# strukturag/libde265

Hardware: AMD Instinct MI355X
Metric: decoded CTBs/s (higher is better)
Workload: dtype u16; 1 GPU; c5_8k10_8tiles; width=7680, height=4320, bit_depth=10, tiles=4x2, ctbs_per_picture=8160, stages=inter+residual+intra+deblock+sao, parallelism=pictures/1

## Files before the change

### libde265_amd/csrc/k_common.h

```cpp
#ifndef M355_K_COMMON_H
#define M355_K_COMMON_H

#include <hip/hip_runtime.h>
#include <stdint.h>

#include "de265_mi355x.h"
#include <k_asm.h>

struct DevRef {
  const void* plane[3];
  int stride[3];
  int valid;
  int pad;
};

struct DevIntraWork {
  uint32_t ctb;
  uint32_t ib_start, ib_count;
  uint16_t nb_same;
  uint16_t nb_earlier;
  uint8_t waves_code;
  uint8_t pad[3];
  uint32_t plan_base;
  uint32_t plan_count;
// ... 273 lines not shown
  uint32_t max_units, n;
  int32_t cf, nhwc, bf16, u16, bdl, bdc;
  float scale[3], bias[3];
  m355_rgb_coeffs k;
  ExportTensorRoi fr[M355_TENSOR_MAX_FRAMES];
  int32_t chroma_loc, pad;
  ColourArgs colour;
};
static_assert(sizeof(ExportTensorRoi) == 88 && sizeof(ExportTensorRoisArgs) <= 4096, "the records of a batch of regions must fit the kernel arguments");
void m355_launch_export_tensor_rois(const ExportTensorRoisArgs& a, int src_bytes, int elem_bytes, int filter, hipStream_t st);

template <class T> __device__ __forceinline__ T d_sel3(int c, T a0, T a1, T a2)
{
  M355_PIN_V(a0); M355_PIN_V(a1); M355_PIN_V(a2);
  return c == 0 ? a0 : (c == 1 ? a1 : a2);
}
#define M355_SEL3(arr, c) d_sel3((c), (arr)[0], (arr)[1], (arr)[2])

#define M355_GATE(p) do { if ((p).timeout[1] == (p).epoch) return; } while (0)

enum { E_TU_V = 1, E_TU_H = 2, E_PB_V = 4, E_PB_H = 8, E_NONZERO = 16 };

struct DevBatch { const DevPic* pics; uint32_t on; };
#define M355_BATCH_PIC_AT(b, k) if (!(((b).on >> (k)) & 1u)) return; const DevPic& p = (b).pics[(k)]
#define M355_BATCH_PIC(b) M355_BATCH_PIC_AT(b, blockIdx.z)
struct HostBatch { const DevPic* host; const DevPic* dev; int n; uint32_t on; };

void m355_launch_validate(const DevPic& p, hipStream_t st);
void m355_launch_meta(const DevPic& p, hipStream_t st);
void m355_launch_clear_gated(const DevPic& p, void* ptr, size_t bytes, hipStream_t st);
void m355_launch_meta_jobs(const DevPic& p, hipStream_t st);
void m355_launch_job_count(const DevPic& p, bool clear_planes, hipStream_t st);
void m355_launch_job_list(const DevPic& p, hipStream_t st);
void m355_launch_meta_planes(const DevPic& p, hipStream_t st, bool cleared, bool with_tu = true);
void m355_launch_meta_planes_jobs(const DevPic& p, hipStream_t st);
void m355_launch_tu_plan(const DevPic& p, hipStream_t st);
void m355_launch_inter(const DevPic& p, bool hbd, hipStream_t st);
#define M355_INTER_TAB_WORDS 300
void m355_inter_tables(bool bytes, int bd_luma, int bd_chroma, uint32_t* out);
void m355_launch_residual(const DevPic& p, bool hbd, bool big, hipStream_t st);
void m355_launch_residual_both(const DevPic& p, bool hbd, hipStream_t st);
void m355_launch_residual_add(const DevPic& p, bool hbd, hipStream_t st);
void m355_launch_residual_tu_plan(const DevPic& p, bool hbd, hipStream_t st);
void m355_launch_intra_plan(const DevPic& p, hipStream_t st);
void m355_launch_intra(const DevPic& p, bool hbd, hipStream_t st, bool ticket_zero = false);
void m355_launch_meta_planes_batch(const HostBatch& b, hipStream_t st);
void m355_launch_residual_batch(const HostBatch& b, bool hbd, bool big, hipStream_t st);
void m355_launch_intra_plan_batch(const HostBatch& b, hipStream_t st);
void m355_launch_deblock_batch(const HostBatch& b, bool hbd, hipStream_t st);
void m355_launch_sao_batch(const HostBatch& b, bool hbd, hipStream_t st);
void m355_launch_intra_batch(const DevPic& first, bool hbd, bool res32, const DevPic* dev_pics, int n, int max_work, uint32_t* ticket, int grid, hipStream_t st);
void m355_launch_deblock(const DevPic& p, bool hbd, hipStream_t st);
void m355_launch_deblock_pass(const DevPic& p, bool hbd, bool vertical, hipStream_t st);
void m355_launch_sao(const DevPic& p, bool hbd, hipStream_t st);
void m355_launch_halo_pack(const DevPic& p, const HaloLayout& h, bool hbd, int which, void* samples, uint32_t* meta, hipStream_t st);
void m355_launch_halo_add(uint32_t* buf, const uint32_t* scratch, uint32_t pitch_words, int n, uint32_t words, hipStream_t st);
void m355_launch_halo_unpack(const DevPic& p, const HaloLayout& h, bool hbd, int which, const void* samples, const uint32_t* meta, hipStream_t st);

__device__ __forceinline__ int d_clip3(int lo, int hi, int v) { return min(max(v, lo), hi); }
__device__ __forceinline__ int d_clip_bd(int v, int bd) { return d_clip3(0, (1 << bd) - 1, v); }
__device__ __forceinline__ int d_abs(int v) { return v < 0 ? -v : v; }
__device__ __forceinline__ int d_sign(int v) { return (v > 0) - (v < 0); }

__device__ __forceinline__ void wave_sync()
{
  __builtin_amdgcn_fence(__ATOMIC_RELEASE, "wavefront");
// ... 19 lines not shown
```

### libde265_amd/csrc/k_meta.hip

```cpp
#include <algorithm>
#include "k_common.h"
#include "k_meta_tu.h"
#include "record_checks.h"

__device__ __forceinline__ void k_meta_cu_body(const DevPic& p, const int blk)
{
  M355_GATE(p);
  const int i = blk * blockDim.x + threadIdx.x;
  if (i >= p.n_cus) return;
  const m355_cu cu = p.cus[i];
  const int x0 = cu.x, y0 = cu.y;
  const int l2m = p.pp.log2_min_cb_size;
  const int n = 1 << (cu.log2_size - l2m);
  const int cx = x0 >> l2m, cy = y0 >> l2m;
  for (int y = cy; y < cy + n && y < p.hcb; y++)
    for (int x = cx; x < cx + n && x < p.wcb; x++) p.cb_cu[y * p.wcb + x] = (uint32_t)i + 1;

  const int ctb_mask = (1 << p.pp.log2_ctb_size) - 1;
  const m355_slice sh = d_slice_at(p, x0, y0);
  int left = x0 != 0, top = y0 != 0;
  if (x0 && (x0 & ctb_mask) == 0) {
    if (!(sh.flags & M355_SF_LF_ACROSS_SLICES) && sh.slice_addr_rs != d_slice_at(p, x0 - 1, y0).slice_addr_rs) left = 0;
    else if (!(p.pp.flags & M355_PF_LF_ACROSS_TILES) && p.tile_id[d_ctb_of(p, x0, y0)] != p.tile_id[d_ctb_of(p, x0 - 1, y0)]) left = 0;
  }
// ... 46 lines not shown
}
__host__ __device__ static inline size_t d_meta_fill16(const DevPic& p) { return ((((size_t)2 * p.w4 * p.h4 + 63) & ~(size_t)63) + (size_t)p.wcb * p.hcb * 4 + 15) / 16; }
__global__ void __launch_bounds__(256) k_job_count(DevPic p, int clear_planes)
{
  M355_GATE(p);
  if (clear_planes) {
    if (blockIdx.x == 0 && threadIdx.x == 0) *p.ticket = 0;
    const size_t n16 = d_meta_fill16(p);
    uint4* q = (uint4*)p.edge_tu;
    for (size_t k = (size_t)blockIdx.x * 256 + threadIdx.x; k < n16; k += (size_t)gridDim.x * 256) q[k] = make_uint4(0, 0, 0, 0);
  }
  const int i = blockIdx.x * 256 + threadIdx.x;
  constexpr int NR = M355_JOB_RANGES;
  int cnt[NR] = {0, 0};
  if (i < p.n_pbs) {
    const m355_pb pb = p.pbs[i];
    const int rng = d_pb_range(p, pb);
    const int n = d_pb_jobs(pb);
#pragma unroll
    for (int k = 0; k < NR; k++) cnt[k] = rng == k ? n : 0;
  }
  __shared__ int s_w[4][NR];
#pragma unroll
  for (int k = 0; k < NR; k++) {
#pragma unroll
    for (int d = 32; d >= 1; d >>= 1) cnt[k] += __shfl_xor(cnt[k], d, 64);
  }
  if ((threadIdx.x & 63) == 0) {
#pragma unroll
    for (int k = 0; k < NR; k++) s_w[threadIdx.x >> 6][k] = cnt[k];
  }
  __syncthreads();
  if (threadIdx.x < NR) p.job_base[blockIdx.x * NR + threadIdx.x] = (uint32_t)(s_w[0][threadIdx.x] + s_w[1][threadIdx.x] + s_w[2][threadIdx.x] + s_w[3][threadIdx.x]);
}
__device__ __forceinline__ void k_meta_pb_body(const DevPic& p, const int chunk, const int n_chunks)
{
  constexpr int NR = M355_JOB_RANGES;
  const int i = chunk * 256 + (int)threadIdx.x;
  const int lane = threadIdx.x & 63;
  const bool active = i < p.n_pbs;
  m355_pb pb;
  if (active) pb = p.pbs[i]; else { pb.x = pb.y = 0; pb.w = pb.h = 0; pb.flags = 0; }
  const int ns = pb.w >> 2;
  const int njobs = active ? d_pb_jobs(pb) : 0;
  const int rng = !active ? NR : d_pb_range(p, pb);
  int incl[NR];
#pragma unroll
  for (int k = 0; k < NR; k++) incl[k] = rng == k ? njobs : 0;
#pragma unroll
  for (int d = 1; d < 64; d <<= 1) {
#pragma unroll
    for (int k = 0; k < NR; k++) { const int t = __shfl_up(incl[k], (unsigned)d, 64); if (lane >= d) incl[k] += t; }
  }
  __shared__ int s_wtot[4][NR];
  const int wave = threadIdx.x >> 6;
  if (lane == 63) {
#pragma unroll
    for (int k = 0; k < NR; k++) s_wtot[wave][k] = incl[k];
  }
  __syncthreads();
  __shared__ uint32_t s_red[4][2 * NR];
  {
    uint32_t acc[2 * NR] = {0, 0, 0, 0};
    for (int ch = (int)threadIdx.x; ch < n_chunks; ch += 256) {
#pragma unroll
      for (int k = 0; k < NR; k++) {
// ... 80 lines not shown
  const int l2w = p.pp.log2_ctb_size - csw, l2h = p.pp.log2_ctb_size - csh;
  const int xC = xCtb << l2w, yC = yCtb << l2h;
  const int ctbSliceAddrRS = d_slice_at(p, min(xC, p.pp.width - 1), min(yC, p.pp.height - 1)).slice_addr_rs;
  const int curFlags = p.slices[p.ctbs[ctb].slice_idx].flags;
  const bool across_tiles = (p.pp.flags & M355_PF_LF_ACROSS_TILES) != 0;
  uint32_t mask = 0;
  for (int k = 0; k < 9; k++) {
    const int nx = xCtb + k % 3 - 1, ny = yCtb + k / 3 - 1;
    bool blocked = true;
    if (nx >= 0 && ny >= 0 && nx < p.ctbW && ny < p.ctbH) {
      const int n = ny * p.ctbW + nx;
      const m355_slice shN = p.slices[p.ctbs[n].slice_idx];
      blocked = (shN.slice_addr_rs < ctbSliceAddrRS && !(curFlags & M355_SF_LF_ACROSS_SLICES)) ||
                (shN.slice_addr_rs > ctbSliceAddrRS && !(shN.flags & M355_SF_LF_ACROSS_SLICES)) ||
                (!across_tiles && p.tile_id[n] != p.tile_id[ctb]);
    }
    if (blocked) mask |= 1u << k;
  }
  if (curFlags & (c == 0 ? M355_SF_SAO_LUMA : M355_SF_SAO_CHROMA)) mask |= 0x8000u;
  p.sao_nb[i] = (uint16_t)mask;
}

void m355_launch_job_count(const DevPic& p, bool clear_planes, hipStream_t st)
{
  if (!p.n_pbs) return;
  hipLaunchKernelGGL(k_job_count, dim3((p.n_pbs + 255) / 256), dim3(256), 0, st, p, clear_planes ? 1 : 0);
}
void m355_launch_job_list(const DevPic& p, hipStream_t st)
{
  if (!p.n_pbs) return;
  const int n_chunks = (p.n_pbs + 255) / 256;
  hipLaunchKernelGGL(k_meta_pb, dim3(n_chunks), dim3(256), 0, st, p);
}
void m355_launch_meta_jobs(const DevPic& p, hipStream_t st)
{
  m355_launch_job_count(p, false, st);
  m355_launch_job_list(p, st);
}

__global__ void __launch_bounds__(256) k_meta_planes(DevPic p, int nb_cu)
{
  const int b = (int)blockIdx.x;
  if (b < nb_cu) k_meta_cu_body(p, b);
  else k_meta_sao_body(p, b - nb_cu);
}
__global__ void __launch_bounds__(256) k_meta_planes_jobs(DevPic p, int nb_pb, int nb_cu)
{
  M355_GATE(p);
  const int b = (int)blockIdx.x;
  if (b < nb_pb) k_meta_pb_body(p, b, nb_pb);
  else if (b < nb_pb + nb_cu) k_meta_cu_body(p, b - nb_pb);
  else k_meta_sao_body(p, b - nb_pb - nb_cu);
}
__global__ void __launch_bounds__(256) k_meta_tu(DevPic p) { k_meta_tu_body(p, (int)blockIdx.x); }
__global__ void __launch_bounds__(256) k_meta_cu_batch(DevBatch b) { M355_BATCH_PIC(b); k_meta_cu_body(p, (int)blockIdx.x); }
__global__ void __launch_bounds__(256) k_meta_tu_batch(DevBatch b) { M355_BATCH_PIC(b); k_meta_tu_body(p, (int)blockIdx.x); }
__global__ void __launch_bounds__(256) k_meta_sao_batch(DevBatch b) { M355_BATCH_PIC(b); k_meta_sao_body(p, (int)blockIdx.x); }
__global__ void __launch_bounds__(256) k_meta_fill_batch(DevBatch b)
{
  M355_BATCH_PIC(b);
  const size_t n16 = d_meta_fill16(p);
  uint4* q = (uint4*)p.edge_tu;
  for (size_t i = (size_t)blockIdx.x * 256 + threadIdx.x; i < n16; i += (size_t)gridDim.x * 256) q[i] = make_uint4(0, 0, 0, 0);
}

void m355_launch_meta_planes(const DevPic& p, hipStream_t st, bool cleared, bool with_tu)
// ... 82 lines not shown
```

### libde265_amd/csrc/runtime.hip

```cpp
#include "runtime_internal.h"

thread_local std::string g_err;
int fail(int code, const char* fmt, ...)
{
  char buf[512];
  va_list ap; va_start(ap, fmt); vsnprintf(buf, sizeof(buf), fmt, ap); va_end(ap);
  g_err = buf;
  return code;
}

extern "C" {
int ev_mark(m355_ctx* c, hipStream_t st, EvRef* out) {
  const unsigned long long t = ++c->ev_ticket;
  m355_ctx::EvSlot& e = c->evring[t % M355_EV_RING];
  if (!e.ev) { if (hipEventCreateWithFlags(&e.ev, hipEventDisableTiming) != hipSuccess) return fail(M355_ERR_HIP, "hipEventCreate failed"); }
  else if (e.ticket) hipEventSynchronize(e.ev);
  if (hipEventRecord(e.ev, st) != hipSuccess) return fail(M355_ERR_HIP, "hipEventRecord failed");
  e.ticket = t;
  out->ticket = t; out->stream = st;
  return M355_OK;
}
void ev_wait(m355_ctx* c, hipStream_t st, const EvRef& r) {
  if (!r.ticket || r.stream == st) return;
  const m355_ctx::EvSlot& e = c->evring[r.ticket % M355_EV_RING];
// ... 12 lines not shown

hipStream_t reader_begin(m355_ctx* c, Frame* f, int kind, const uint32_t** gate, uint32_t* epoch) {
  const hipStream_t st = f->wr_stream ? f->wr_stream : lane(c).stream;
  if (!f->wr_stream) ev_wait(c, st, f->wr);
  ev_wait(c, st, f->reader[kind]);
  if (!gate) return st;
  if (f->wr_stream && f->wr_gate) { *gate = f->wr_gate; *epoch = f->wr_epoch; }
  else {
    *gate = lane(c).timeout; *epoch = ++c->epoch;
    if (*epoch == 0) *epoch = ++c->epoch;
  }
  return st;
}
int reader_end(m355_ctx* c, Frame* f, int kind, hipStream_t st) { return ev_mark(c, st, &f->reader[kind]); }
void readers_wait(m355_ctx* c, hipStream_t st, const Frame* f) {
  for (const EvRef& m : f->reader) ev_wait(c, st, m);
}

int lane_class_priority(int index) {
  static int lo = 0, hi = 0, probed = 0;
  if (!probed) { probed = 1; if (hipDeviceGetStreamPriorityRange(&lo, &hi) != hipSuccess) lo = hi = 0; }
  const int cls = (index / 3) % 3;
  return cls == 0 ? 0 : (cls == 1 ? hi : lo);
}
int lane_priorities_mode() { return 2; }
static int lane_priority(int index) { return lane_priorities_mode() == 1 ? lane_class_priority(index) : 0; }
static int lane_create(m355_ctx* c, Lane& l, int index)
{
  HIPCHK(hipStreamCreateWithPriority(&l.stream, hipStreamNonBlocking, lane_priority(index)));
  HIPCHK(hipStreamCreateWithPriority(&l.stream2, hipStreamNonBlocking, lane_priority(index)));
  HIPCHK(hipEventCreateWithFlags(&l.ev_fork, hipEventDisableTiming));
  HIPCHK(hipEventCreateWithFlags(&l.ev_fork2, hipEventDisableTiming));
  HIPCHK(hipEventCreateWithFlags(&l.ev_join, hipEventDisableTiming));
  HIPCHK(hipMalloc(&l.ticket, 64));
  HIPCHK(hipMalloc(&l.timeout, 128));
  HIPCHK(hipMemsetAsync(l.ticket, 0, 64, l.stream));
  HIPCHK(hipMemsetAsync(l.timeout, 0, 128, l.stream));
  HIPCHK(hipMemsetAsync(l.timeout + 2, 0xFF, 8, l.stream));
  HIPCHK(hipStreamSynchronize(l.stream));
  return M355_OK;
}
static void lane_destroy(Lane& l)
{
  if (l.stream) hipStreamSynchronize(l.stream);
  if (l.stream2) hipStreamSynchronize(l.stream2);
  if (l.work.used) frame_free(l.work);
  void* bufs[] = {l.pb_of, l.edge, l.ticket, l.timeout, l.edge_tu, l.cuf, l.resbuf, l.jobs, l.sao_nb, l.iplan, l.job_base};
  for (void* b : bufs) if (b) hipFree(b);
  if (l.ev_fork) hipEventDestroy(l.ev_fork);
  if (l.ev_fork2) hipEventDestroy(l.ev_fork2);
  if (l.ev_join) hipEventDestroy(l.ev_join);
  if (l.stream_hi) { hipStreamSynchronize(l.stream_hi); hipStreamDestroy(l.stream_hi); }
  if (l.stream2) hipStreamDestroy(l.stream2);
  if (l.stream) hipStreamDestroy(l.stream);
  l = Lane();
}
hipError_t sync_all(m355_ctx* c) {
  hipError_t e = hipSuccess;
  auto sync = [&](hipStream_t s) { if (s) { hipError_t e2 = hipStreamSynchronize(s); if (e == hipSuccess) e = e2; } };
  for (const Lane& l : c->lanes) { sync(l.stream); sync(l.stream_hi); }
  for (hipStream_t bs : c->batch_stream) sync(bs);
  sync(c->maps_stream);
  return e;
}


static std::vector<TileRect> rank_tiles(const m355_pic_params& pp, int rank, int nranks)
{
  std::vector<TileRect> v;
  const int cs = 1 << pp.log2_ctb_size, n_tiles = pp.num_tile_cols * pp.num_tile_rows;
  for (int ty = 0, t = 0; ty < pp.num_tile_rows; ty++)
    for (int tx = 0; tx < pp.num_tile_cols; tx++, t++) {
      if (m355_shard_owner_of_tile(t, n_tiles, nranks) != rank) continue;
      TileRect r = {pp.col_bd[tx] * cs, pp.row_bd[ty] * cs, pp.col_bd[tx + 1] * cs, pp.row_bd[ty + 1] * cs};
      if (r.x1 > pp.width) r.x1 = pp.width;
      if (r.y1 > pp.height) r.y1 = pp.height;
      v.push_back(r);
    }
  return v;
}
static size_t tiles_bytes(const m355_pic_params& pp, const std::vector<TileRect>& v)
{
  const int cf = pp.chroma_format_idc;
  const int sw = (cf == 1 || cf == 2) ? 2 : 1, sh = cf == 1 ? 2 : 1;
// ... 933 lines not shown
```

### libde265_amd/csrc/runtime_decode.hip

```cpp
#include "runtime_internal.h"

extern "C" {

bool chain_residuals_forced();

int prepare(m355_ctx* c, Resident& r, DevPic& d_out, bool& want_sao_out, hipStream_t st) {
  hipSetDevice(c->device);
  const m355_picture& pic = r.hdr;
  const m355_pic_params& pp = pic.pp;
  Frame* dst = get_frame(c, pic.dst_frame);
  if (!dst) return fail(M355_ERR_INVALID, "dst_frame %d is not a live frame", pic.dst_frame);
  if (dst->w != pp.width || dst->h != pp.height || dst->cf != pp.chroma_format_idc || dst->bdl != pp.bit_depth_luma || dst->bdc != pp.bit_depth_chroma)
    return fail(M355_ERR_INVALID, "dst frame geometry does not match the picture parameters");
  DevPic d = r.dp;
  d.ref_valid = 0;
  DevRef refs[M355_MAX_REF_FRAMES];
  memset(refs, 0, sizeof(refs));
  for (int i = 0; i < M355_MAX_REF_FRAMES; i++) {
    if (pic.ref_frames[i] < 0) continue;
    Frame* f = get_frame(c, pic.ref_frames[i]);
    if (!f) return fail(M355_ERR_INVALID, "ref_frames[%d]=%d is not a live frame", i, pic.ref_frames[i]);
    if (f->w != dst->w || f->h != dst->h || f->cf != dst->cf || f->bdl != dst->bdl || f->bdc != dst->bdc)
      return fail(M355_ERR_INVALID, "reference frame %d geometry differs (motion.cc:377-398 would conceal; record FILL instead)", i);
    if (f == dst) return fail(M355_ERR_INVALID, "a picture cannot reference itself");
    for (int cc = 0; cc < 3; cc++) { refs[i].plane[cc] = f->plane[cc]; refs[i].stride[cc] = f->stride[cc]; }
    refs[i].valid = 1;
    d.ref_valid |= 1u << i;
  }
  if (!r.refs_dev) {
    HIPCHK(hipMalloc(&r.refs_dev, sizeof(refs)));
    HIPCHK(hipHostMalloc(&r.refs_host, sizeof(refs), hipHostMallocDefault));
    r.refs_valid = false;
  }
  if (!r.refs_valid || memcmp(r.refs_host, refs, sizeof(refs)) != 0) {
    if (!r.fresh) HIPCHK(sync_all(c));
    memcpy(r.refs_host, refs, sizeof(refs));
    HIPCHK(hipMemcpyAsync(r.refs_dev, r.refs_host, sizeof(refs), hipMemcpyHostToDevice, st));
// ... 5 lines not shown
    const uint32_t* tab = nullptr;
    for (auto& e : c->inter_tabs) if (e.first == key) tab = e.second;
    if (!tab) {
      uint32_t host[M355_INTER_TAB_WORDS];
      m355_inter_tables(dst->bpp[0] == 1, std::min((int)pp.bit_depth_luma, 16), std::min((int)pp.bit_depth_chroma, 16), host);
      uint32_t* dev = nullptr;
      HIPCHK(hipMalloc(&dev, sizeof(host)));
      HIPCHK(hipMemcpy(dev, host, sizeof(host), hipMemcpyHostToDevice));
      c->inter_tabs.emplace_back(key, dev);
      tab = dev;
    }
    d.inter_tabs = tab;
  }
  Lane& L = lane(c);
  int rc;
  {
    const size_t u4 = (size_t)d.w4 * d.h4, ncb = (size_t)d.wcb * d.hcb;
    const size_t need = ((2 * u4 + 63) & ~(size_t)63) + ncb * 4 + 64;
    if ((rc = grow(&L.edge_tu, &L.cap_u4, need, st, false))) return rc;
    if ((rc = grow(&L.pb_of, &L.cap_cb, u4, st, true))) return rc;
  }
  {
    size_t n = 0;
    for (int cc = 0; cc < 3; cc++) {
      d.edge_col_ofs[cc] = (uint32_t)n; n += (size_t)d.ctbW * (size_t)(dst->ph[cc] >> 1);
      d.edge_row_ofs[cc] = (uint32_t)n; n += (size_t)d.ctbH * (size_t)(dst->pw[cc] >> 1);
    }
    if ((rc = grow(&L.edge, &L.cap_edge, n + 1, st, true))) return rc;
  }
  if ((rc = grow(&L.cuf, &L.cap_cuf, (size_t)pic.n_cus + (size_t)r.halo.n_units + 1, st, false))) return rc;
  const size_t res_intra = (((size_t)pic.res_len + 64) & ~(size_t)63) * (m355_res32(pp) ? 2 : 1);
  size_t res_tiles = 0;
  for (int s = 0; s < 4; s++) { d.res_tile_base[s] = (uint32_t)res_tiles; res_tiles += (size_t)pic.rb_count[s] << (2 * (s + 2)); }
  const bool tiles = (c->depth >= sched::chain_residual_tiles_min_depth || chain_residuals_forced()) && (long long)pic.pp.width * pic.pp.height <= sched::one_stream_max_samples;
  const size_t res_need = res_intra + (tiles ? res_tiles : 0) + 1;
  if ((rc = grow(&L.resbuf, &L.cap_res, res_need, st, false))) return rc;
  d.res_tiles = tiles ? L.resbuf + res_intra : nullptr;
  d.res_front = 0;
  if ((rc = grow(&L.sao_nb, &L.cap_sao, (size_t)d.nCtb * 3, st, false))) return rc;
  {
    const size_t area = (size_t)pp.width * pp.height;
    const size_t cap = pic.n_pbs > 0 ? std::min(area / 16, area / 32 + 8 * (size_t)pic.n_pbs) + 256 : 1;
    const size_t n_chunks = ((size_t)(pic.n_pbs > 0 ? pic.n_pbs : 0) + 255) / 256;
    if ((rc = grow(&L.jobs, &L.cap_jobs, cap, st, false))) return rc;
    if ((rc = grow(&L.job_base, &L.cap_jobbase, n_chunks * M355_JOB_RANGES + 8, st, true))) return rc;
    d.jobs_cap = (uint32_t)cap; d.job_base = L.job_base; d.job_tot = L.job_base + n_chunks * M355_JOB_RANGES;
  }
  if ((rc = grow(&L.iplan, &L.cap_iplan, (size_t)r.n_iplan + 8, st, false))) return rc;

  const bool want_sao = (c->stages & M355_STAGE_SAO) && (pp.flags & M355_PF_SAO_ENABLED);
  Frame* target = dst;
  if (want_sao) {
    if (!L.work.used || L.work.w != dst->w || L.work.h != dst->h || L.work.cf != dst->cf || L.work.bdl != dst->bdl || L.work.bdc != dst->bdc) {
      HIPCHK(sync_all(c));
      if (L.work.used) frame_free(L.work);
      frame_geometry(L.work, dst->w, dst->h, dst->cf, dst->bdl, dst->bdc);
      if ((rc = frame_alloc(L.work, st))) return rc;
    }
    target = &L.work;
  }
  for (int cc = 0; cc < 3; cc++) {
    d.pw[cc] = dst->pw[cc]; d.ph[cc] = dst->ph[cc];
    d.plane[cc] = target->plane[cc]; d.stride[cc] = target->stride[cc];
    d.out_plane[cc] = dst->plane[cc]; d.out_stride[cc] = dst->stride[cc];
  }
  d.edge_tu = L.edge_tu; d.edge_pb = L.edge_tu + (size_t)d.w4 * d.h4;
  d.cb_cu = (uint32_t*)(L.edge_tu + (((size_t)2 * d.w4 * d.h4 + 63) & ~(size_t)63));
  d.cuf = L.cuf; d.pb_of = L.pb_of;
  d.fill_pb_of_in_meta = ((c->stages & M355_STAGE_INTER) && m355_inter_uses_jobs(d)) ? 0 : 1;
  d.jobs = L.jobs; d.sao_nb = L.sao_nb; d.iplan = L.iplan;
  d.resbuf = L.resbuf; d.edge = L.edge; d.ticket = L.ticket; d.timeout = L.timeout;
  {
    static const int grid_env = getenv("M355_INTRA_GRID") ? atoi(getenv("M355_INTRA_GRID")) : 0;
    static int slots = 0;
    if (!slots) { hipDeviceProp_t prop; slots = (hipGetDeviceProperties(&prop, c->device) == hipSuccess && prop.multiProcessorCount > 0) ? 2 * prop.multiProcessorCount : 512; }
    d.intra_grid = grid_env > 0 ? grid_env : std::max(64, slots / std::max(1, c->depth));
    d.intra_keeper = c->depth <= sched::intra_keeper_max_depth;
    if (!d.intra_keeper && r.dp.intra_dense) {
      bool idle = true;
      for (int i = 0; i < c->depth && idle; i++) if (&c->lanes[i] != &L && ev_query(c, c->lanes[i].last) != hipSuccess) idle = false;
      d.intra_keeper = idle;
    }
    static const bool no_keeper = getenv("M355_TEST_NO_KEEPER") != nullptr;
    if (no_keeper) d.intra_keeper = 0;
    static const int halo_late = getenv("M355_TEST_HALO_LATE") ? atoi(getenv("M355_TEST_HALO_LATE")) : 0;
    d.test_halo_late = halo_late;
  }
  d.epoch = ++c->epoch;
  if (d.epoch == 0) d.epoch = ++c->epoch;
  c->dbg_intra[0] = r.n_intra_work; c->dbg_intra[1] = r.n_intra_ticket; c->dbg_intra[2] = r.n_intra_heavy; c->dbg_intra[3] = r.n_intra_light;
  d_out = d; want_sao_out = want_sao;
  return M355_OK;
}

void clear_target(m355_ctx* c, const DevPic& d, Frame* tgt, bool gated, hipStream_t st) {
  for (int cc = 0; cc < 3; cc++) {
    if (!tgt->pw[cc]) continue;
    const size_t bytes = (size_t)tgt->stride[cc] * tgt->ph[cc] * tgt->bpp[cc];
    if (gated) m355_launch_clear_gated(d, tgt->plane[cc], bytes, st);
    else hipMemsetAsync(tgt->plane[cc], 0, bytes, st);
  }
}

bool chain_residuals_forced() { static const bool on = getenv("M355_TEST_CHAIN_RESIDUALS") != nullptr; return on; }

hipStream_t launch_prediction(m355_ctx* c, const Resident& r, const DevPic& d, bool hbd, hipStream_t st, hipEvent_t* ev, bool with_intra, hipStream_t chain, Frame* hazard_dst) {
  Lane& L = lane(c);
  const bool single = d.intra_dense || (long long)d.pp.width * d.pp.height <= sched::one_stream_max_samples;
  hipStream_t s2 = single ? st : L.stream2;
  static const int clear_min = getenv("M355_CLEAR_IN_COUNT_MIN") ? atoi(getenv("M355_CLEAR_IN_COUNT_MIN")) : sched::clear_in_count_min_pbs;
  const bool clear_in_count = d.n_pbs >= std::max(1, clear_min);
  bool tu_plan_with_residuals = false;
  const bool res_front = (chain || chain_residuals_forced()) && d.res_tiles && (c->stages & M355_STAGE_RESIDUAL) && d.pp.bit_depth_luma <= 15 && d.pp.bit_depth_chroma <= 15 &&
                         d.rb_count[0] + d.rb_count[1] + d.rb_count[2] + d.rb_count[3] > 0;
  if (clear_in_count) m355_launch_job_count(d, true, st);
  if (!single) { hipEventRecord(L.ev_fork, st); hipStreamWaitEvent(s2, L.ev_fork, 0); }
  if (single && clear_in_count && (c->stages & M355_STAGE_INTRA)) {
    m355_launch_meta_planes_jobs(d, st);
    if (c->depth <= sched::tu_plan_in_residuals_max_depth && (c->stages & M355_STAGE_RESIDUAL) && !res_front) tu_plan_with_residuals = true; else m355_launch_tu_plan(d, st);
  } else {
    if (c->stages & M355_STAGE_INTRA) {
      m355_launch_meta_planes(d, s2, clear_in_count, false);
      m355_launch_tu_plan(d, s2);
    } else m355_launch_meta_planes(d, s2, clear_in_count);
    if (clear_in_count) m355_launch_job_list(d, st); else m355_launch_meta_jobs(d, st);
  }
  auto launch_residuals = [&](const DevPic& dd) {
    hipStream_t sr = !single ? s2 : st;
    if (sr != st) { hipEventRecord(L.ev_fork2, st); hipStreamWaitEvent(s2, L.ev_fork2, 0); }
    if (tu_plan_with_residuals) m355_launch_residual_tu_plan(dd, hbd, st);
    else if (sr == st) m355_launch_residual_both(dd, hbd, st);
    else {
      m355_launch_residual(dd, hbd, false, sr);
      m355_launch_residual(dd, hbd, true, st);
    }
  };
  if (res_front) { DevPic dq = d; dq.res_front = 1; launch_residuals(dq); }
  if (ev) hipEventRecord(ev[1], st);
  if (chain && chain != st) {
    EvRef front;
    if (ev_mark(c, st, &front) == M355_OK) {
      st = chain; ev_wait(c, st, front);
      if (ev) hipEventRecord(ev[1], st);
    }
  }
  if (hazard_dst) dst_hazards(c, hazard_dst, true, st);
  if (c->depth >= 2)
    for (int i = 0; i < M355_MAX_REF_FRAMES; i++) {
      Frame* f = r.hdr.ref_frames[i] >= 0 ? get_frame(c, r.hdr.ref_frames[i]) : nullptr;
      if (f) ev_wait(c, st, f->wr);
    }
  if (c->stages & M355_STAGE_INTER) m355_launch_inter(d, hbd, st);
  if (ev) hipEventRecord(ev[2], st);
  if ((c->stages & M355_STAGE_RESIDUAL) && !res_front) launch_residuals(d);
  else if (res_front) m355_launch_residual_add(d, hbd, st);
  if (!single) { hipEventRecord(L.ev_join, s2); hipStreamWaitEvent(st, L.ev_join, 0); }
  if (ev) hipEventRecord(ev[3], st);
  if (with_intra && (c->stages & M355_STAGE_INTRA)) m355_launch_intra(d, hbd, st, clear_in_count);
  if (ev) hipEventRecord(ev[4], st);
  return st;
}

void dst_hazards(m355_ctx* c, Frame* dstf, bool piped, hipStream_t st) {
  readers_wait(c, st, dstf);
  if (!piped) return;
  ev_wait(c, st, dstf->wr);
  for (int k = 0; k < M355_MAX_LANES; k++) ev_wait(c, st, dstf->rd[k]);
}

int mark_done(m355_ctx* c, Resident& r, Frame* dstf, hipStream_t st, const DevPic* d) {
  const int rc = ev_mark(c, st, &r.done);
  if (rc) return rc;
  r.fresh = false;
  dstf->wr_stream = st; dstf->wr = r.done;
  dstf->wr_gate = d ? d->timeout : nullptr; dstf->wr_epoch = d ? d->epoch : 0;
  lane(c).last = r.done; lane(c).last_stream = st;
  return M355_OK;
}

struct DecodeState {
  DevPic d; bool want_sao = false; hipEvent_t* ev = nullptr;
  hipStream_t st = nullptr;
};

enum { PRE_ALL = 0, PRE_NO_INTRA = 1, PRE_HAZARDS = 2 };
static int decode_pre(m355_ctx* c, Resident& r, bool rotate, DecodeState& S, int mode, hipStream_t on_stream = nullptr)
{
  const bool with_intra = mode == PRE_ALL;
  if (r.sharded) return fail(M355_ERR_INVALID, "a sharded picture is decoded by phases (m355_decode_phase)");
  hipStream_t chain = nullptr;
  if (rotate && c->depth >= 2) {
// ... 94 lines not shown
  if (e != hipSuccess) return fail(M355_ERR_HIP, "kernel launch failed: %s", hipGetErrorString(e));
  {
    static const bool dbg = getenv("M355_DEBUG_TIMEOUT") && atoi(getenv("M355_DEBUG_TIMEOUT"));
    if (dbg) {
      hipStreamSynchronize(st);
      uint32_t t = 0;
      hipMemcpy(&t, lane(c).timeout, 4, hipMemcpyDeviceToHost);
      if (t) fprintf(stderr, "m355: decode %llu (epoch %u, %d pbs, %d ibs, %d cus, lane %d): intra wait gave up\n", c->serial, d.epoch, d.n_pbs, d.n_ibs, d.n_cus, c->active);
    }
  }
  return M355_OK;
}

int decode(m355_ctx* c, Resident& r, bool rotate) {
  DecodeState S;
  const int rc = decode_pre(c, r, rotate, S, PRE_ALL);
  return rc ? rc : decode_post(c, r, S);
}

int status_of(m355_ctx* c, m355_ctx::Status& s) {
  if (!s.validated) return M355_OK;
  const uint32_t* w = c->status_words + 4 * (s.serial % M355_STATUS_RING);
  if (w[1] != s.epoch) return M355_OK;
  const unsigned long long key = (unsigned long long)w[2] | ((unsigned long long)w[3] << 32);
  uint32_t bad = (uint32_t)key;
  if ((uint32_t)(key >> 32) != ~s.epoch) bad = 0;
  static const char* const names[8] = {"?", "cu", "tu", "pb", "weight", "rb", "ib", "?"};
  s.reported = true;
  return fail(M355_ERR_INVALID, "picture %llu: %s %u rejected by the device-side list validation (the picture was not decoded)", s.serial, names[(bad >> 28) & 7], bad & 0x0FFFFFFFu);
}

unsigned long long m355_last_serial(m355_ctx* c) { return c->serial; }
M355_API void m355_debug_intra_counts(m355_ctx* c, int* out) { for (int i = 0; i < 4; i++) out[i] = c->dbg_intra[i]; }

int m355_decode_status(m355_ctx* c, unsigned long long serial)
{
  if (serial == 0 || serial > c->serial) return fail(M355_ERR_INVALID, "no decode with serial %llu", serial);
  m355_ctx::Status& s = c->status[serial % M355_STATUS_RING];
  if (s.serial != serial) return fail(M355_ERR_STALE, "decode %llu is older than the last %d decodes: its status is no longer kept (m355_wait reports rejections)", serial, M355_STATUS_RING);
  hipSetDevice(c->device);
  const hipError_t q = ev_query(c, s.done);
  if (q == hipErrorNotReady) return M355_ERR_BUSY;
  if (q != hipSuccess) return fail(M355_ERR_HIP, "hipEventQuery failed: %s", hipGetErrorString(q));
  return status_of(c, s);
}

int m355_decode_batch(m355_ctx* c, const int* handles, int n)
{
  if (n < 1 || !handles) return fail(M355_ERR_INVALID, "m355_decode_batch: no pictures");
  if (n > std::max(1, c->depth)) return fail(M355_ERR_INVALID, "m355_decode_batch: %d pictures on %d lanes (m355_set_pipeline_depth)", n, c->depth);
  for (int k = 0; k < n; k++) {
    const int h = handles[k];
    if (h < 0 || h >= (int)c->resident.size() || !c->resident[h].used) return fail(M355_ERR_INVALID, "bad picture handle");
    for (int j = 0; j < k; j++) if (handles[j] == h) return fail(M355_ERR_INVALID, "m355_decode_batch: picture %d twice in one batch", h);
    const Resident& r = c->resident[h];
    const m355_pic_params &a = r.hdr.pp, &b = c->resident[handles[0]].hdr.pp;
    if (r.sharded) return fail(M355_ERR_INVALID, "a sharded picture is decoded by phases (m355_decode_phase)");
    if (!r.dp.intra_dense || r.dp.n_pbs > 0) return fail(M355_ERR_INVALID, "m355_decode_batch: picture %d is not an intra picture", h);
    if (a.chroma_format_idc != b.chroma_format_idc || (a.bit_depth_luma > 8) != (b.bit_depth_luma > 8))
      return fail(M355_ERR_INVALID, "m355_decode_batch: the pictures differ in chroma format or sample type");
    for (int j = 0; j < k; j++)
      if (c->resident[handles[j]].hdr.dst_frame == r.hdr.dst_frame) return fail(M355_ERR_INVALID, "m355_decode_batch: two pictures into frame %d", r.hdr.dst_frame);
  }
  hipSetDevice(c->device);
  if (n == 1 || !(c->stages & M355_STAGE_INTRA)) {
    for (int k = 0; k < n; k++) { int rc = decode(c, c->resident[handles[k]]); if (rc) return rc; }
// ... 85 lines not shown
```

### libde265_amd/csrc/runtime_internal.h

```cpp
#ifndef M355_RUNTIME_INTERNAL_H
#define M355_RUNTIME_INTERNAL_H
#include <dlfcn.h>
#include <stdarg.h>
#include <stdio.h>
#include <stdlib.h>
#include <string.h>

#include <algorithm>
#include <array>
#include <atomic>
#include <chrono>
#include <condition_variable>
#include <functional>
#include <mutex>
#include <thread>
#include <string>
#include <utility>
#include <vector>

#include <pthread.h>
#include "k_common.h"
#include "k_hash.h"
#include "k_measure.h"
#include "k_stats.h"
#include "k_ssim.h"
#include "k_msssim.h"
#include "k_maps.h"


extern thread_local std::string g_err;
int fail(int code, const char* fmt, ...);
#define HIPCHK(call) do { hipError_t e_ = (call); if (e_ != hipSuccess) return fail(M355_ERR_HIP, "%s failed: %s", #call, hipGetErrorString(e_)); } while (0)

#define M355_STATUS_RING 64
#define M355_BATCH_RING 16
#define M355_MAX_LANES 32
#define M355_TRANSIENT_MAX 12

namespace sched {
constexpr long long one_stream_max_samples = 16ll << 20;
constexpr int clear_in_count_min_pbs = 64 * 256;
constexpr int tu_plan_in_residuals_max_depth = 1;
constexpr int intra_keeper_max_depth = 1;
constexpr int chain_split_min_depth = 3;
constexpr int chain_residual_tiles_min_depth = 3;
constexpr int intra_class_first_lane = 3;
constexpr bool intra_light_32x32 = false;
}

struct EvRef { unsigned long long ticket = 0; hipStream_t stream = nullptr; };
#define M355_EV_RING 256

enum ReaderKind { RD_DOWNLOAD, RD_EXPORT, RD_HASH, RD_MEASURE, RD_STATS, RD_SSIM, RD_MSSSIM, RD_KINDS };
struct Frame {
  bool used = false;
  int w = 0, h = 0, cf = 0, bdl = 0, bdc = 0;
  int pw[3] = {0, 0, 0}, ph[3] = {0, 0, 0}, stride[3] = {0, 0, 0}, bpp[3] = {1, 1, 1};
  void* plane[3] = {nullptr, nullptr, nullptr};
  EvRef wr, rd[M355_MAX_LANES];
  hipStream_t wr_stream = nullptr;
  const uint32_t* wr_gate = nullptr; uint32_t wr_epoch = 0;
  EvRef reader[RD_KINDS];
};

static void frame_geometry(Frame& f, int w, int h, int cf, int bdl, int bdc)
{
  f.w = w; f.h = h; f.cf = cf; f.bdl = bdl; f.bdc = bdc;
  const int sw = (cf == 1 || cf == 2) ? 2 : 1, sh = (cf == 1) ? 2 : 1;
  for (int c = 0; c < 3; c++) {
    f.bpp[c] = ((c ? bdc : bdl) <= 8) ? 1 : 2;
    if (c && cf == 0) { f.pw[c] = f.ph[c] = f.stride[c] = 0; continue; }
    f.pw[c] = c ? w / sw : w;
    f.ph[c] = c ? h / sh : h;
    const int pitch_bytes = (f.pw[c] * f.bpp[c] + 127) & ~127;
    f.stride[c] = pitch_bytes / f.bpp[c];
  }
}
static int frame_alloc(Frame& f, hipStream_t st)
{
  for (int c = 0; c < 3; c++) {
// ... 29 lines not shown
  int n_intra_ticket = 0, n_intra_heavy = 0, n_intra_light = 0;
  uint32_t n_iplan = 0;
  bool sharded = false;
  int shard_rank = 0, shard_n = 1;
  HaloLayout halo;
  DevPic live;
  bool live_sao = false, live_valid = false;
  void* xprev = nullptr;
  int lane = 0;
  void* xb[4] = {nullptr, nullptr, nullptr, nullptr};
  size_t xb_bytes[4] = {0, 0, 0, 0};
  void* xscratch = nullptr;
  std::vector<hipEvent_t> x3_read;
  unsigned long long xb_epoch = 0;
  std::vector<int> peers;
  EvRef up;
  EvRef done;
  EvRef maps;
  bool fresh = false;
  bool arena = false;
  m355_arena_caps caps;
  int arena_halo_units = 0;
  bool reserved = false;
  bool device_validate = false;
  size_t xscratch_pitch = 0;
  std::vector<uint8_t> sched_u8;
  std::vector<uint32_t> sched_u32;
  std::vector<uint32_t> sched_order, sched_cand, sched_bucket, sched_u32b;
};

struct Lane {
  hipStream_t stream = nullptr, stream2 = nullptr;
  hipEvent_t ev_fork = nullptr, ev_fork2 = nullptr, ev_join = nullptr;
  hipStream_t stream_hi = nullptr, last_stream = nullptr;
  EvRef last;
  Frame work;
  uint32_t *pb_of = nullptr, *ticket = nullptr, *timeout = nullptr;
  unsigned long long* edge = nullptr;
  uint8_t *edge_tu = nullptr, *cuf = nullptr;
  int16_t* resbuf = nullptr;
  uint32_t* jobs = nullptr;
  uint16_t* sao_nb = nullptr;
  uint16_t* iplan = nullptr;
  uint32_t* job_base = nullptr;
  size_t cap_cb = 0, cap_u4 = 0, cap_edge = 0, cap_cuf = 0, cap_res = 0, cap_jobs = 0, cap_sao = 0, cap_iplan = 0, cap_jobbase = 0;
};

struct m355_ctx {
  int device = 0;
  Lane lanes[M355_MAX_LANES];
  int depth = 1, active = 0;
  std::vector<std::pair<uint32_t, uint32_t*>> inter_tabs;
  struct EvSlot { hipEvent_t ev = nullptr; unsigned long long ticket = 0; };
  EvSlot evring[M355_EV_RING];
  unsigned long long ev_ticket = 0;
  std::vector<Frame> frames;
  std::vector<Resident> resident;
  Resident transient[M355_TRANSIENT_MAX];
  int next_transient = 0;
  int last_transient = -1;
  int transient_ring() const { return 3; }
  uint32_t epoch = 0;
  struct Status { unsigned long long serial = 0; uint32_t epoch = 0; bool validated = false, reported = false; EvRef done; };
  Status status[M355_STATUS_RING];
  uint32_t* status_words = nullptr;
  unsigned long long serial = 0;
  unsigned long long lost_first = 0; int lost_count = 0;
  int stages = M355_STAGE_ALL;
  int dbg_intra[4] = {0, 0, 0, 0};
  int shard_rank = 0, shard_n = 0;
  m355_comm comm = {nullptr, nullptr, nullptr};
  void* rccl = nullptr;
  void* ipc = nullptr;
  int xchg_h = -1, xchg_k = -1;
  std::vector<hipEvent_t> evs;
  int ev_used = 0;
  bool timing_on = false;
  uint32_t* hash_acc = nullptr;
  struct HashSlot {
    unsigned long long ticket = 0; int type = 0, np = 0;
    int row_bytes[3] = {0, 0, 0}, rows[3] = {0, 0, 0};
    EvRef mark; int frame = -1;
    uint8_t* planes = nullptr; size_t planes_cap = 0;
  };
  HashSlot hash_slot[M355_HASH_REQUESTS];
  unsigned long long hash_ticket = 0;
  uint32_t *hash_rec = nullptr, *hash_res = nullptr;
  std::vector<std::pair<uint8_t*, size_t>> hash_pool;
  struct MeasSlot {
    unsigned long long ticket = 0;
    int np = 0, pw[3] = {0, 0, 0}, ph[3] = {0, 0, 0}, row0[3] = {0, 0, 0};
    EvRef mark; int frame[2] = {-1, -1};
    unsigned long long* rows = nullptr; size_t rows_cap = 0;
  };
  MeasSlot meas_slot[M355_MEASURE_REQUESTS];
  unsigned long long meas_ticket = 0;
  unsigned long long *meas_rec = nullptr, *meas_res = nullptr;
  std::vector<std::pair<unsigned long long*, size_t>> meas_pool;
  struct StatsSlot {
    unsigned long long ticket = 0;
    int np = 0, light = 0;
// ... 173 lines not shown
```

Baseline: 26.85 million CTB64/s.

## Build inter job lists ahead on second stream, overlapping previous picture's inter

For large pictures decoded on two streams at depth 1, the job count and job list kernels now run on the secondary stream once the previous picture's inter stage has finished, instead of on the main stream ahead of this picture's inter. A new clear kernel resets the ticket and edge/TU planes on the main stream in their place. Inter then waits on an event for the jobs. This is meant to take job-list construction off the critical path by overlapping it with earlier work, at the cost of extra events, epoch tracking and several guard conditions.

```diff
diff --git a/libde265_amd/csrc/k_common.h b/libde265_amd/csrc/k_common.h
--- a/libde265_amd/csrc/k_common.h
+++ b/libde265_amd/csrc/k_common.h
@@ -329,6 +329,7 @@
 void m355_launch_meta_jobs(const DevPic& p, hipStream_t st);
 void m355_launch_job_count(const DevPic& p, bool clear_planes, hipStream_t st);
 void m355_launch_job_list(const DevPic& p, hipStream_t st);
+void m355_launch_meta_clear(const DevPic& p, hipStream_t st);
 void m355_launch_meta_planes(const DevPic& p, hipStream_t st, bool cleared, bool with_tu = true);
 void m355_launch_meta_planes_jobs(const DevPic& p, hipStream_t st);
 void m355_launch_tu_plan(const DevPic& p, hipStream_t st);
diff --git a/libde265_amd/csrc/k_meta.hip b/libde265_amd/csrc/k_meta.hip
--- a/libde265_amd/csrc/k_meta.hip
+++ b/libde265_amd/csrc/k_meta.hip
@@ -102,6 +102,14 @@
   }
   __syncthreads();
   if (threadIdx.x < NR) p.job_base[blockIdx.x * NR + threadIdx.x] = (uint32_t)(s_w[0][threadIdx.x] + s_w[1][threadIdx.x] + s_w[2][threadIdx.x] + s_w[3][threadIdx.x]);
+}
+__global__ void __launch_bounds__(256) k_meta_clear(DevPic p)
+{
+  M355_GATE(p);
+  if (blockIdx.x == 0 && threadIdx.x == 0) *p.ticket = 0;
+  const size_t n16 = d_meta_fill16(p);
+  uint4* q = (uint4*)p.edge_tu;
+  for (size_t k = (size_t)blockIdx.x * 256 + threadIdx.x; k < n16; k += (size_t)gridDim.x * 256) q[k] = make_uint4(0, 0, 0, 0);
 }
 __device__ __forceinline__ void k_meta_pb_body(const DevPic& p, const int chunk, const int n_chunks)
 {
@@ -248,6 +256,11 @@
   const int n_chunks = (p.n_pbs + 255) / 256;
   hipLaunchKernelGGL(k_meta_pb, dim3(n_chunks), dim3(256), 0, st, p);
 }
+void m355_launch_meta_clear(const DevPic& p, hipStream_t st)
+{
+  const unsigned grid = (unsigned)std::min<size_t>((d_meta_fill16(p) + 1023) / 1024 + 1, 1024);
+  hipLaunchKernelGGL(k_meta_clear, dim3(grid), dim3(256), 0, st, p);
+}
 void m355_launch_meta_jobs(const DevPic& p, hipStream_t st)
 {
   m355_launch_job_count(p, false, st);
diff --git a/libde265_amd/csrc/runtime.hip b/libde265_amd/csrc/runtime.hip
--- a/libde265_amd/csrc/runtime.hip
+++ b/libde265_amd/csrc/runtime.hip
@@ -68,6 +68,8 @@
   HIPCHK(hipEventCreateWithFlags(&l.ev_fork, hipEventDisableTiming));
   HIPCHK(hipEventCreateWithFlags(&l.ev_fork2, hipEventDisableTiming));
   HIPCHK(hipEventCreateWithFlags(&l.ev_join, hipEventDisableTiming));
+  HIPCHK(hipEventCreateWithFlags(&l.ev_inter, hipEventDisableTiming));
+  HIPCHK(hipEventCreateWithFlags(&l.ev_jobs, hipEventDisableTiming));
   HIPCHK(hipMalloc(&l.ticket, 64));
   HIPCHK(hipMalloc(&l.timeout, 128));
   HIPCHK(hipMemsetAsync(l.ticket, 0, 64, l.stream));
@@ -86,6 +88,8 @@
   if (l.ev_fork) hipEventDestroy(l.ev_fork);
   if (l.ev_fork2) hipEventDestroy(l.ev_fork2);
   if (l.ev_join) hipEventDestroy(l.ev_join);
+  if (l.ev_inter) hipEventDestroy(l.ev_inter);
+  if (l.ev_jobs) hipEventDestroy(l.ev_jobs);
   if (l.stream_hi) { hipStreamSynchronize(l.stream_hi); hipStreamDestroy(l.stream_hi); }
   if (l.stream2) hipStreamDestroy(l.stream2);
   if (l.stream) hipStreamDestroy(l.stream);
diff --git a/libde265_amd/csrc/runtime_decode.hip b/libde265_amd/csrc/runtime_decode.hip
--- a/libde265_amd/csrc/runtime_decode.hip
+++ b/libde265_amd/csrc/runtime_decode.hip
@@ -3,6 +3,7 @@
 extern "C" {
 
 bool chain_residuals_forced();
+bool two_stream_lane_forced();
 
 int prepare(m355_ctx* c, Resident& r, DevPic& d_out, bool& want_sao_out, hipStream_t st) {
   hipSetDevice(c->device);
@@ -74,7 +75,8 @@
   const size_t res_intra = (((size_t)pic.res_len + 64) & ~(size_t)63) * (m355_res32(pp) ? 2 : 1);
   size_t res_tiles = 0;
   for (int s = 0; s < 4; s++) { d.res_tile_base[s] = (uint32_t)res_tiles; res_tiles += (size_t)pic.rb_count[s] << (2 * (s + 2)); }
-  const bool tiles = (c->depth >= sched::chain_residual_tiles_min_depth || chain_residuals_forced()) && (long long)pic.pp.width * pic.pp.height <= sched::one_stream_max_samples;
+  const bool tiles = (c->depth >= sched::chain_residual_tiles_min_depth || chain_residuals_forced()) && (long long)pic.pp.width * pic.pp.height <= sched::one_stream_max_samples &&
+                     !two_stream_lane_forced();
   const size_t res_need = res_intra + (tiles ? res_tiles : 0) + 1;
   if ((rc = grow(&L.resbuf, &L.cap_res, res_need, st, false))) return rc;
   d.res_tiles = tiles ? L.resbuf + res_intra : nullptr;
@@ -84,8 +86,10 @@
     const size_t area = (size_t)pp.width * pp.height;
     const size_t cap = pic.n_pbs > 0 ? std::min(area / 16, area / 32 + 8 * (size_t)pic.n_pbs) + 256 : 1;
     const size_t n_chunks = ((size_t)(pic.n_pbs > 0 ? pic.n_pbs : 0) + 255) / 256;
+    const size_t cap_jobs0 = L.cap_jobs, cap_jobbase0 = L.cap_jobbase;
     if ((rc = grow(&L.jobs, &L.cap_jobs, cap, st, false))) return rc;
     if ((rc = grow(&L.job_base, &L.cap_jobbase, n_chunks * M355_JOB_RANGES + 8, st, true))) return rc;
+    if (L.cap_jobs != cap_jobs0 || L.cap_jobbase != cap_jobbase0) L.jobs_grown = true;
     d.jobs_cap = (uint32_t)cap; d.job_base = L.job_base; d.job_tot = L.job_base + n_chunks * M355_JOB_RANGES;
   }
   if ((rc = grow(&L.iplan, &L.cap_iplan, (size_t)r.n_iplan + 8, st, false))) return rc;
@@ -130,6 +134,7 @@
   }
   d.epoch = ++c->epoch;
   if (d.epoch == 0) d.epoch = ++c->epoch;
+  L.epoch_prev = L.epoch_cur; L.epoch_cur = d.epoch;
   c->dbg_intra[0] = r.n_intra_work; c->dbg_intra[1] = r.n_intra_ticket; c->dbg_intra[2] = r.n_intra_heavy; c->dbg_intra[3] = r.n_intra_light;
   d_out = d; want_sao_out = want_sao;
   return M355_OK;
@@ -145,27 +150,47 @@
 }
 
 bool chain_residuals_forced() { static const bool on = getenv("M355_TEST_CHAIN_RESIDUALS") != nullptr; return on; }
+bool two_stream_lane_forced() { static const bool on = getenv("M355_TEST_TWO_STREAM_LANE") != nullptr; return on; }
 
 hipStream_t launch_prediction(m355_ctx* c, const Resident& r, const DevPic& d, bool hbd, hipStream_t st, hipEvent_t* ev, bool with_intra, hipStream_t chain, Frame* hazard_dst) {
   Lane& L = lane(c);
-  const bool single = d.intra_dense || (long long)d.pp.width * d.pp.height <= sched::one_stream_max_samples;
+  const bool two_stream_size = (long long)d.pp.width * d.pp.height > sched::one_stream_max_samples || two_stream_lane_forced();
+  const bool single = d.intra_dense || !two_stream_size;
   hipStream_t s2 = single ? st : L.stream2;
+  static const int ahead_env = getenv("M355_JOBS_AHEAD") ? atoi(getenv("M355_JOBS_AHEAD")) : -1;
+  const bool ahead_on = ahead_env >= 0 ? ahead_env != 0 : c->depth <= sched::jobs_ahead_max_depth;
+  const bool plain = !chain && with_intra && !r.sharded;
+  const bool grown = L.jobs_grown;
+  L.jobs_grown = false;
+  const bool ahead = ahead_on && !single && plain && (c->stages & M355_STAGE_INTER) && !d.fill_pb_of_in_meta && d.n_pbs > 0 && !r.device_validate && !grown &&
+                     L.epoch_inter != 0 && L.epoch_inter == L.epoch_prev && st == L.stream && (!L.last_stream || L.last_stream == L.stream);
   static const int clear_min = getenv("M355_CLEAR_IN_COUNT_MIN") ? atoi(getenv("M355_CLEAR_IN_COUNT_MIN")) : sched::clear_in_count_min_pbs;
   const bool clear_in_count = d.n_pbs >= std::max(1, clear_min);
   bool tu_plan_with_residuals = false;
   const bool res_front = (chain || chain_residuals_forced()) && d.res_tiles && (c->stages & M355_STAGE_RESIDUAL) && d.pp.bit_depth_luma <= 15 && d.pp.bit_depth_chroma <= 15 &&
                          d.rb_count[0] + d.rb_count[1] + d.rb_count[2] + d.rb_count[3] > 0;
-  if (clear_in_count) m355_launch_job_count(d, true, st);
+  if (ahead) {
+    ev_wait(c, s2, r.up);
+    hipStreamWaitEvent(s2, L.ev_inter, 0);
+    m355_launch_job_count(d, false, s2);
+    m355_launch_job_list(d, s2);
+    hipEventRecord(L.ev_jobs, s2);
+    m355_launch_meta_clear(d, st);
+    c->n_jobs_ahead++;
+  } else if (clear_in_count) m355_launch_job_count(d, true, st);
+  const bool cleared = clear_in_count || ahead;
   if (!single) { hipEventRecord(L.ev_fork, st); hipStreamWaitEvent(s2, L.ev_fork, 0); }
   if (single && clear_in_count && (c->stages & M355_STAGE_INTRA)) {
     m355_launch_meta_planes_jobs(d, st);
     if (c->depth <= sched::tu_plan_in_residuals_max_depth && (c->stages & M355_STAGE_RESIDUAL) && !res_front) tu_plan_with_residuals = true; else m355_launch_tu_plan(d, st);
   } else {
     if (c->stages & M355_STAGE_INTRA) {
-      m355_launch_meta_planes(d, s2, clear_in_count, false);
+      m355_launch_meta_planes(d, s2, cleared, false);
       m355_launch_tu_plan(d, s2);
-    } else m355_launch_meta_planes(d, s2, clear_in_count);
-    if (clear_in_count) m355_launch_job_list(d, st); else m355_launch_meta_jobs(d, st);
+    } else m355_launch_meta_planes(d, s2, cleared);
+    if (ahead) {}
+    else if (clear_in_count) m355_launch_job_list(d, st);
+    else m355_launch_meta_jobs(d, st);
   }
   auto launch_residuals = [&](const DevPic& dd) {
     hipStream_t sr = !single ? s2 : st;
@@ -192,13 +217,15 @@
       Frame* f = r.hdr.ref_frames[i] >= 0 ? get_frame(c, r.hdr.ref_frames[i]) : nullptr;
       if (f) ev_wait(c, st, f->wr);
     }
+  if (ahead) hipStreamWaitEvent(st, L.ev_jobs, 0);
   if (c->stages & M355_STAGE_INTER) m355_launch_inter(d, hbd, st);
+  if (ahead_on && plain && two_stream_size) { hipEventRecord(L.ev_inter, st); L.epoch_inter = d.epoch; }
   if (ev) hipEventRecord(ev[2], st);
   if ((c->stages & M355_STAGE_RESIDUAL) && !res_front) launch_residuals(d);
   else if (res_front) m355_launch_residual_add(d, hbd, st);
   if (!single) { hipEventRecord(L.ev_join, s2); hipStreamWaitEvent(st, L.ev_join, 0); }
   if (ev) hipEventRecord(ev[3], st);
-  if (with_intra && (c->stages & M355_STAGE_INTRA)) m355_launch_intra(d, hbd, st, clear_in_count);
+  if (with_intra && (c->stages & M355_STAGE_INTRA)) m355_launch_intra(d, hbd, st, cleared);
   if (ev) hipEventRecord(ev[4], st);
   return st;
 }
@@ -359,6 +386,7 @@
 
 unsigned long long m355_last_serial(m355_ctx* c) { return c->serial; }
 M355_API void m355_debug_intra_counts(m355_ctx* c, int* out) { for (int i = 0; i < 4; i++) out[i] = c->dbg_intra[i]; }
+M355_API unsigned long long m355_debug_jobs_ahead(m355_ctx* c) { return c->n_jobs_ahead; }
 
 int m355_decode_status(m355_ctx* c, unsigned long long serial)
 {
diff --git a/libde265_amd/csrc/runtime_internal.h b/libde265_amd/csrc/runtime_internal.h
--- a/libde265_amd/csrc/runtime_internal.h
+++ b/libde265_amd/csrc/runtime_internal.h
@@ -46,6 +46,7 @@
 constexpr int chain_residual_tiles_min_depth = 3;
 constexpr int intra_class_first_lane = 3;
 constexpr bool intra_light_32x32 = false;
+constexpr int jobs_ahead_max_depth = 1;
 }
 
 struct EvRef { unsigned long long ticket = 0; hipStream_t stream = nullptr; };
@@ -141,6 +142,9 @@
 struct Lane {
   hipStream_t stream = nullptr, stream2 = nullptr;
   hipEvent_t ev_fork = nullptr, ev_fork2 = nullptr, ev_join = nullptr;
+  hipEvent_t ev_inter = nullptr, ev_jobs = nullptr;
+  uint32_t epoch_cur = 0, epoch_prev = 0, epoch_inter = 0;
+  bool jobs_grown = false;
   hipStream_t stream_hi = nullptr, last_stream = nullptr;
   EvRef last;
   Frame work;
@@ -176,6 +180,7 @@
   unsigned long long serial = 0;
   unsigned long long lost_first = 0; int lost_count = 0;
   int stages = M355_STAGE_ALL;
+  unsigned long long n_jobs_ahead = 0;
   int dbg_intra[4] = {0, 0, 0, 0};
   int shard_rank = 0, shard_n = 0;
   m355_comm comm = {nullptr, nullptr, nullptr};
```

New measurement: 26.84 million CTB64/s, median of 2. About the same (-0.0%).
